# DichenZhang1/libultrahdr_dev

Hardware: AMD Instinct MI355X
Metric: MPixels/sec gain-map generate+apply, 4K P010 batch (higher is better)
Workload: dtype u8/u16 in, f32+f64 math, u8/u32 out

## Files before the change

### libultrahdr_dev_amd/csrc/uhdr_capi.hip

```cpp
#include <hip/hip_runtime.h>

#include <algorithm>
#include <memory>
#include <cmath>
#include <cstdio>
#include <cstring>
#include <map>
#include <chrono>
#include <mutex>
#include <thread>
#include <tuple>
#include <vector>

#include "../../include/uhdr_hip.h"
#include "uhdr_kernels.h"
#include "uhdr_jpeg.h"
#include "uhdr_jpegr.h"

namespace {

using namespace uhdr;

thread_local char t_err[256] = "";

// ... 369 lines not shown
  c.log2_min_d = std::log2((double)md.minContentBoost);
  c.log2_max_d = std::log2((double)md.maxContentBoost);
  c.idw = idw;
  c.lut = nullptr;
  c.lut_boost_factor = c.display_boost > 0 ? c.display_boost / md.maxContentBoost : 1.0f;
  const double lut_top = std::exp2(std::fmax(c.log2_min_d, c.log2_max_d) * (double)c.lut_boost_factor) / (double)c.display_boost;
  c.lut_plain_div = (c.display_boost >= 0x1p-20f && c.display_boost <= 0x1p20f && std::fabs(c.log2_min_d * (double)c.lut_boost_factor) <= 40.0 &&
                     std::fabs(c.log2_max_d * (double)c.lut_boost_factor) <= 40.0 && lut_top <= 32768.0) ? 1u : 0u;
  const double ratio = (double)c.display_boost / (double)md.maxContentBoost;
  c.fast.A = (float)((c.log2_max_d - c.log2_min_d) * ratio);
  c.fast.B = (float)(c.log2_min_d * ratio - std::log2((double)c.display_boost));
  c.fast.A255 = (float)((c.log2_max_d - c.log2_min_d) * ratio / 255.0);
  std::vector<float> t;
  build_idw_tables(4, t);
  for (int oy = 0; oy < 4; ++oy)
    for (int pr = 0; pr < 2; ++pr)
      for (int k = 1; k < 4; ++k)
        for (int j = 0; j < 2; ++j)
          c.fast.wD[oy][pr][k - 1][j] = t[oy * 16 + (2 * pr + j) * 4 + k];
  c.tab = nullptr;
  c.ex_ws = nullptr;
  c.ex_cap = 0;
  c.cells_per_thread = 8;
  c.step_x = c.step_y = 0;
  return c;
}
AppImage app_image(const uhdr_hip_image_t& yuv, const uhdr_hip_image_t& map, void* dst) {
  AppImage a;
  a.y = static_cast<const uint8_t*>(yuv.data);
  a.u = static_cast<const uint8_t*>(yuv.chroma_data);
  a.v = a.u + yuv.chroma_stride * (yuv.height / 2);
  a.map = static_cast<const uint8_t*>(map.data);
  a.dst = dst;
  a.y_stride = (uint32_t)yuv.luma_stride;
  a.c_stride = (uint32_t)yuv.chroma_stride;
  return a;
}
bool app_fast_s4(const AppConsts& c, const AppImage& a) {
  if ((uint64_t)a.y_stride * c.height >= (1ull << 32) || (uint64_t)c.width * c.height >= (1ull << 29)) return false;
  return c.scale == 4 && c.width == 4u * c.map_w && c.height == 4u * c.map_h && al(a.y, 4) && a.y_stride % 4u == 0 &&
         al(a.u, 2) && al(a.v, 2) && a.c_stride % 2u == 0 && al(a.dst, 16);
}
void fill_apply_dest(const uhdr_hip_image_t* yuv, uhdr_hip_image_t* dest) {
  dest->width = yuv->width;
  dest->height = yuv->height;
  dest->colorGamut = yuv->colorGamut;
}
// ... 3485 lines not shown
```

### libultrahdr_dev_amd/csrc/uhdr_kernels.h

```cpp
#pragma once
#include <hip/hip_runtime_api.h>
#include <stdint.h>

namespace uhdr {

constexpr uint32_t kStatSlotWaves = 1024, kStatSlotPlain = 15, kStatSlotSaved = 4, kStatSlotWords = 16 + 16 * kStatSlotSaved;
constexpr uint32_t kStatLists = 64, kStatCap = 252, kStatEst = 8 + kStatLists, kStatSlotCnt = kStatEst + 2 * kStatLists,
                   kStatHdr = kStatSlotCnt + kStatSlotWaves,
                   kStatWords = kStatHdr + (kStatLists * kStatCap > kStatSlotWaves * kStatSlotWords ? kStatLists * kStatCap : kStatSlotWaves * kStatSlotWords);
static_assert(kStatHdr % 4u == 0u && kStatSlotWords % 4u == 0u && kStatWords % 4u == 0u, "saved entries are read and written as 16-byte pieces");
constexpr int kMaxChunk = 64;

constexpr uint32_t kLutSrgbInvN = 1024, kLutHlgInvN = 4096, kLutPqInvN = 4096, kLutHlgN = 65536, kLutPqN = 65536;
constexpr uint32_t kLutSrgbInv = 0, kLutHlgInv = kLutSrgbInv + kLutSrgbInvN, kLutPqInv = kLutHlgInv + kLutHlgInvN,
                   kLutHlg = kLutPqInv + kLutPqInvN, kLutPq = kLutHlg + kLutHlgN, kLutTotal = kLutPq + kLutPqN;
constexpr uint32_t kTabS1Bytes = 0x3C00 + 16;
constexpr uint32_t kTabS1PowBytes = 512u * 8u;
constexpr uint32_t kTabS2Cells = 129, kTabS2Floats = 260;
constexpr uint32_t kTabS2LdsBytes = kTabS2Cells * 256u;
constexpr uint32_t kTabS1Lin = kLutTotal, kTabS1Hlg = kTabS1Lin + kTabS1Bytes / 4, kTabS1Pq = kTabS1Hlg + kTabS1PowBytes / 4,
                   kTabS2Hlg = kTabS1Pq + kTabS1PowBytes / 4, kTabS2Pq = kTabS2Hlg + kTabS2Floats, kTabEnd = kTabS2Pq + kTabS2Floats;
constexpr uint32_t kCodeHlg = kTabEnd, kCodePq = kCodeHlg + kLutHlgN / 2, kLutBufferFloats = kCodePq + kLutPqN / 2;
constexpr uint32_t kGainLutN = 1024;

// ... 25 lines not shown
  uint32_t enc_byte_min, enc_byte_max;
  const float* lut;
  double log2_min_d, log2_max_d;
};
struct GenImage {
  const uint8_t* y;
  const uint8_t* u;
  const uint16_t* hy;
  const uint16_t* huv;
  uint8_t* map;
  uint32_t y_stride, c_stride, hy_stride, huv_stride;
};
struct GenBatch {
  GenImage img[kMaxChunk];
};

struct AppFast {
  float A, B, A255;
  float wD[4][2][3][2];
};
struct AppConsts {
  uint32_t width, height, map_w, map_h, scale;
  uint32_t cells_per_thread;
  uint32_t step_x, step_y;
  float display_boost, inv_display_boost, max_boost, inv_max_boost;
  double log2_min_d, log2_max_d;
  const float* idw;
  const float* lut;
  const float* tab;
  float lut_boost_factor;
  uint32_t lut_plain_div;
  uint32_t* ex_ws;
  uint32_t ex_cap;
  AppFast fast;
};
constexpr uint32_t kExLists = 1024;
constexpr uint32_t kExHdrWords = 8 + kExLists;
inline size_t ex_ws_bytes(uint32_t cap) { return ((size_t)kMaxChunk * kExHdrWords + (size_t)kMaxChunk * kExLists * cap) * 4u; }
inline uint32_t ex_list_cap(uint64_t pixels) { return (uint32_t)(pixels / 16u / kExLists) + 64u; }
struct AppImage {
  const uint8_t* y;
  const uint8_t* u;
  const uint8_t* v;
  const uint8_t* map;
  void* dst;
  uint32_t y_stride, c_stride;
};
// ... 107 lines not shown
```

### libultrahdr_dev_amd/csrc/uhdr_kernels.hip

```cpp
#include "uhdr_kernels.h"

#include <hip/hip_runtime.h>

#include <algorithm>
#include <cmath>

#include "uhdr_device_math.h"
#include "uhdr_wave_scan.h"

namespace uhdr {

__constant__ float c_idw4[4 * 64];

__constant__ float c_idw4p[64];

hipError_t upload_idw4(const float* tables) {
  float p[64];
  for (int oy = 0; oy < 4; ++oy)
    for (int pr = 0; pr < 2; ++pr)
      for (int k = 0; k < 4; ++k)
        for (int h = 0; h < 2; ++h) p[((oy * 2 + pr) * 4 + k) * 2 + h] = tables[oy * 16 + (2 * pr + h) * 4 + k];
  hipError_t e = hipMemcpyToSymbol(HIP_SYMBOL(c_idw4p), p, sizeof(p));
  if (e != hipSuccess) return e;
  return hipMemcpyToSymbol(HIP_SYMBOL(c_idw4), tables, sizeof(float) * 4 * 64);
// ... 277 lines not shown
    out[k] = encode_gain_guarded(gain[k], c.min_boost, c.max_boost, c.log2_min, c.log2_max, c.enc_scale, c.enc_byte_min,
                                 c.enc_byte_max);
  return 3u;
}

typedef uint32_t u32x4 __attribute__((ext_vector_type(4)));
typedef uint32_t u32x2 __attribute__((ext_vector_type(2)));
__device__ __forceinline__ uint4 ld_stream(const uint4* p) {
  const u32x4 v = __builtin_nontemporal_load(reinterpret_cast<const u32x4*>(p));
  return make_uint4(v.x, v.y, v.z, v.w);
}
__device__ __forceinline__ uint2 ld_stream(const uint2* p) {
  const u32x2 v = __builtin_nontemporal_load(reinterpret_cast<const u32x2*>(p));
  return make_uint2(v.x, v.y);
}
__device__ __forceinline__ uint32_t ld_stream(const uint32_t* p) {
  return __builtin_nontemporal_load(p);
}
__device__ __forceinline__ void st_stream(uint4* p, uint4 v) {
  __builtin_nontemporal_store((u32x4){v.x, v.y, v.z, v.w}, reinterpret_cast<u32x4*>(p));
}
__device__ __forceinline__ void st_stream(uint2* p, uint2 v) {
  __builtin_nontemporal_store((u32x2){v.x, v.y}, reinterpret_cast<u32x2*>(p));
}
__device__ __forceinline__ uint32_t ld8(const uint8_t* p) { return *p; }
__device__ __forceinline__ uint32_t ld16(const uint16_t* p) { return *p; }

constexpr int kGenBlock = 256, kGenTiles = 4;

template <bool ALIGNED>
__device__ __forceinline__ void load_pair(const GenConsts& c, const GenImage& im, const uint8_t* im_v, uint32_t my, uint32_t pr,
                                          bool two, uint32_t (&hy)[2][4][2], uint32_t (&huv)[2][2][2], uint32_t (&y8)[2][4],
                                          uint32_t (&u8)[2][2], uint32_t (&v8)[2][2]) {
  const uint32_t mx = pr * 2u;
  if (ALIGNED) {
    const uint32_t hoff = 4u * my * im.hy_stride + 8u * pr, yoff = 4u * my * im.y_stride + 8u * pr;
#pragma unroll
    for (int r = 0; r < 4; ++r) {
      const uint4 q = ld_stream(reinterpret_cast<const uint4*>(im.hy + (hoff + r * im.hy_stride)));
      hy[0][r][0] = q.x; hy[0][r][1] = q.y; hy[1][r][0] = q.z; hy[1][r][1] = q.w;
      const uint2 p = ld_stream(reinterpret_cast<const uint2*>(im.y + (yoff + r * im.y_stride)));
      y8[0][r] = p.x; y8[1][r] = p.y;
    }
    const uint32_t huvoff = 2u * my * im.huv_stride + 8u * pr, coff = 2u * my * im.c_stride + 4u * pr;
#pragma unroll
    for (int r = 0; r < 2; ++r) {
// ... 602 lines not shown
  asm("v_lshl_or_b32 %0, %1, 10, %2" : "=v"(t) : "v"(__float_as_uint(g)), "v"(__float_as_uint(r)));
  asm("v_lshl_or_b32 %0, %1, 20, %2" : "=v"(t) : "v"(__float_as_uint(b)), "v"(t));
  return t;
}

template <int K>
__device__ __forceinline__ float cvt_byte(uint32_t w) { return (float)((w >> (8 * K)) & 0xffu); }

struct PairF { f2 c[3]; f2 factor; float2 e[6]; };
struct PairM { f2 s[3]; float2 e[6]; };
struct ChromaRow { f2 crv, ngs, cbu; };
__device__ __forceinline__ ChromaRow chroma_row(uint32_t uu, uint32_t vv) {
  constexpr float kCrS = kP3Cr * k255, kCbS = kP3Cb * k255, kGCbS = kP3GCb * k255, kGCrS = kP3GCr * k255;
  const f2 uf = (f2){cvt_byte<0>(uu), cvt_byte<1>(uu)};
  const f2 vf = (f2){cvt_byte<0>(vv), cvt_byte<1>(vv)};
  ChromaRow o;
  o.crv = pk_fma(vf, splat(kCrS), splat(-128.0f * kCrS));
  o.cbu = pk_fma(uf, splat(kCbS), splat(-128.0f * kCbS));
  o.ngs = pk_fma(uf, splat(-kGCbS), pk_fma(vf, splat(-kGCrS), splat(128.0f * kGCbS + 128.0f * kGCrS)));
  return o;
}
template <int FMT>
__device__ __forceinline__ void apply_cell_piped(const AppConsts& c, void* dst, uint32_t cx, uint32_t cy,
                                                 const uint32_t (&yrow)[4], const uint32_t (&uu)[2], const uint32_t (&vv)[2],
                                                 float m1, float m2, float m3, float m4, uint32_t slot8, const char* lut) {
  typedef ApplyTab<FMT, false> T;
  ChromaRow cr = chroma_row(uu[0], vv[0]);
  const float a255 = c.fast.A255;
  f2 d23 = (f2){m2 - m1, m3 - m1}, d4b = (f2){m4 - m1, __builtin_fmaf(m1, a255, c.fast.B)};
  asm("" : "+v"(d23), "+v"(d4b));
  PairF pf[2];
  PairM pm[2];
  uint32_t px[4];
#pragma unroll
  for (int k = 0; k < 10; ++k) {
    if (k < 8) {
      const int oy = k >> 1, pr = k & 1;
      const f2 w1 = (f2){c.fast.wD[oy][pr][0][0], c.fast.wD[oy][pr][0][1]}, w2 = (f2){c.fast.wD[oy][pr][1][0], c.fast.wD[oy][pr][1][1]};
      const f2 w3 = (f2){c.fast.wD[oy][pr][2][0], c.fast.wD[oy][pr][2][1]};
      if (k == 4) cr = chroma_row(uu[1], vv[1]);
      PairF& f = pf[k & 1];
      const f2 E = pk_fma(bc_lo(d4b), w3, pk_fma(bc_hi(d23), w2, pk_fma(bc_lo(d23), w1, bc_hi(d4b))));
      const f2 yraw = pr ? (f2){cvt_byte<2>(yrow[oy]), cvt_byte<3>(yrow[oy])} : (f2){cvt_byte<0>(yrow[oy]), cvt_byte<1>(yrow[oy])};
      if (pr) {
        f.c[0] = pk_fma_sat_bc<1>(yraw, splat(k255), cr.crv); f.c[1] = pk_fma_sat_bc<1>(yraw, splat(k255), cr.ngs);
        f.c[2] = pk_fma_sat_bc<1>(yraw, splat(k255), cr.cbu);
      } else {
// ... 14 lines not shown
        asm("v_fma_f32 %0, %1, %2, %3" : "=v"(t.x) : "v"(f.e[2 * ch].y), "v"(f.c[ch].x), "v"(f.e[2 * ch].x));
        asm("v_fma_f32 %0, %1, %2, %3" : "=v"(t.y) : "v"(f.e[2 * ch + 1].y), "v"(f.c[ch].y), "v"(f.e[2 * ch + 1].x));
        m.s[ch] = pk_fma(t, f.factor, splat(2.0f));
      }
#pragma unroll
      for (int ch = 0; ch < 3; ++ch) {
        m.e[2 * ch] = *reinterpret_cast<const float2*>(lut + T::kS2Base + s2_address(m.s[ch].x, slot8));
        m.e[2 * ch + 1] = *reinterpret_cast<const float2*>(lut + T::kS2Base + s2_address(m.s[ch].y, slot8));
      }
    }
    __builtin_amdgcn_sched_barrier(0);
    if (k >= 2) {
      const int q = k - 2, oy = q >> 1, pr = q & 1;
      PairM& m = pm[q & 1];
      float o[6];
#pragma unroll
      for (int ch = 0; ch < 3; ++ch) {
        asm("v_fma_f32 %0, %1, %2, %3" : "=v"(o[2 * ch]) : "v"(m.e[2 * ch].y), "v"(m.s[ch].x), "v"(m.e[2 * ch].x));
        asm("v_fma_f32 %0, %1, %2, %3" : "=v"(o[2 * ch + 1]) : "v"(m.e[2 * ch + 1].y), "v"(m.s[ch].y), "v"(m.e[2 * ch + 1].x));
      }
      px[2 * pr] = pack10_bits(o[0], o[2], o[4]);
      px[2 * pr + 1] = pack10_bits(o[1], o[3], o[5]);
      if (pr) {
        const uint32_t off = ((4u * cy + oy) * c.width + 4u * cx) * 4u;
        st_stream(reinterpret_cast<uint4*>(static_cast<char*>(dst) + off), make_uint4(px[0], px[1], px[2], px[3]));
      }
    }
    __builtin_amdgcn_sched_barrier(0);
  }
}

constexpr uint32_t kXchSecond = 72;
constexpr uint32_t kXchPerWave = 136;
template <int FMT, bool MASK>
__device__ __forceinline__ void apply_cell_piped1(const AppConsts& c, const AppImage& im, uint32_t cx, uint32_t cy,
                                                  const uint32_t (&yrow)[4], const uint32_t (&uu)[2], const uint32_t (&vv)[2],
                                                  float m1, float m2, float m3, float m4, const char* lut, uint4* xch) {
  ChromaRow cr = chroma_row(uu[0], vv[0]);
  const float a255 = c.fast.A255;
  f2 d23 = (f2){m2 - m1, m3 - m1}, d4b = (f2){m4 - m1, __builtin_fmaf(m1, a255, c.fast.B)};
  asm("" : "+v"(d23), "+v"(d4b));
  PairF pf[2];
  PairOut po[2];
  const uint32_t lane = threadIdx.x & 63u;
#pragma unroll
  for (int k = 0; k < 9; ++k) {
    if (k < 8) {
      const int oy = k >> 1, pr = k & 1;
      const f2 w1 = (f2){c.fast.wD[oy][pr][0][0], c.fast.wD[oy][pr][0][1]}, w2 = (f2){c.fast.wD[oy][pr][1][0], c.fast.wD[oy][pr][1][1]};
      const f2 w3 = (f2){c.fast.wD[oy][pr][2][0], c.fast.wD[oy][pr][2][1]};
      if (k == 4) cr = chroma_row(uu[1], vv[1]);
      PairF& f = pf[k & 1];
      const f2 E = pk_fma(bc_lo(d4b), w3, pk_fma(bc_hi(d23), w2, pk_fma(bc_lo(d23), w1, bc_hi(d4b))));
      const f2 yraw = pr ? (f2){cvt_byte<2>(yrow[oy]), cvt_byte<3>(yrow[oy])} : (f2){cvt_byte<0>(yrow[oy]), cvt_byte<1>(yrow[oy])};
      if (pr) {
        f.c[0] = pk_fma_sat_bc<1>(yraw, splat(k255), cr.crv); f.c[1] = pk_fma_sat_bc<1>(yraw, splat(k255), cr.ngs);
        f.c[2] = pk_fma_sat_bc<1>(yraw, splat(k255), cr.cbu);
      } else {
        f.c[0] = pk_fma_sat_bc<0>(yraw, splat(k255), cr.crv); f.c[1] = pk_fma_sat_bc<0>(yraw, splat(k255), cr.ngs);
        f.c[2] = pk_fma_sat_bc<0>(yraw, splat(k255), cr.cbu);
      }
      f.factor = exp2_2(E);
#pragma unroll
      for (int ch = 0; ch < 3; ++ch) tab_pair<0>(f.c[ch], lut, f.e[2 * ch], f.e[2 * ch + 1]);
    }
    __builtin_amdgcn_sched_barrier(0);
    if (k >= 1) {
      const int q = k - 1, oy = q >> 1, pr = q & 1;
      PairF& f = pf[q & 1];
      f2 lin[3];
#pragma unroll
      for (int ch = 0; ch < 3; ++ch) {
        f2 t;
        asm("v_fma_f32 %0, %1, %2, %3" : "=v"(t.x) : "v"(f.e[2 * ch].y), "v"(f.c[ch].x), "v"(f.e[2 * ch].x));
        asm("v_fma_f32 %0, %1, %2, %3" : "=v"(t.y) : "v"(f.e[2 * ch + 1].y), "v"(f.c[ch].y), "v"(f.e[2 * ch + 1].x));
        lin[ch] = oetf2_scaled<FMT>(t * f.factor);
      }
      po[pr].r = lin[0]; po[pr].g = lin[1]; po[pr].b = lin[2];
      if (pr) {
        const uint32_t pix0 = (4u * cy + oy) * c.width + 4u * cx;
        if (FMT == 2 || FMT == 3) {
          uint4 o;
          o.x = pack10_scaled<MASK>(po[0].r.x, po[0].g.x, po[0].b.x); o.y = pack10_scaled<MASK>(po[0].r.y, po[0].g.y, po[0].b.y);
          o.z = pack10_scaled<MASK>(po[1].r.x, po[1].g.x, po[1].b.x); o.w = pack10_scaled<MASK>(po[1].r.y, po[1].g.y, po[1].b.y);
          st_stream(reinterpret_cast<uint4*>(static_cast<uint32_t*>(im.dst) + pix0), o);
        } else if (FMT == 1) {
          const uint2 a = pack_f16_hw(po[0].r.x, po[0].g.x, po[0].b.x), bb = pack_f16_hw(po[0].r.y, po[0].g.y, po[0].b.y);
          const uint2 cc = pack_f16_hw(po[1].r.x, po[1].g.x, po[1].b.x), d = pack_f16_hw(po[1].r.y, po[1].g.y, po[1].b.y);
          if (xch != nullptr) {
            xch[lane] = make_uint4(a.x, a.y, bb.x, bb.y);
            xch[kXchSecond + lane] = make_uint4(cc.x, cc.y, d.x, d.y);
            __builtin_amdgcn_wave_barrier();
            const uint32_t from = (lane & 1u) * kXchSecond + (lane >> 1);
            const uint4 s0 = xch[from], s1 = xch[from + 32u];
            __builtin_amdgcn_wave_barrier();
            uint4* o = reinterpret_cast<uint4*>(static_cast<uint2*>(im.dst) + (uint32_t)__builtin_amdgcn_readfirstlane((int)pix0));
            st_stream(o + lane, s0);
            st_stream(o + 64u + lane, s1);
          } else {
            uint4* o = reinterpret_cast<uint4*>(static_cast<uint2*>(im.dst) + pix0);
            o[0] = make_uint4(a.x, a.y, bb.x, bb.y);
            o[1] = make_uint4(cc.x, cc.y, d.x, d.y);
          }
        } else {
          const size_t plane = (size_t)c.width * c.height;
          uint16_t* base16 = static_cast<uint16_t*>(im.dst);
          const f2 ch[3][2] = {{po[0].r, po[1].r}, {po[0].g, po[1].g}, {po[0].b, po[1].b}};
#pragma unroll
          for (int p = 0; p < 3; ++p) {
            const uint32_t q0 = 0x3ffu & (uint32_t)ch[p][0].x, q1 = 0x3ffu & (uint32_t)ch[p][0].y;
            const uint32_t q2 = 0x3ffu & (uint32_t)ch[p][1].x, q3 = 0x3ffu & (uint32_t)ch[p][1].y;
            st_stream(reinterpret_cast<uint2*>(base16 + p * plane + pix0), make_uint2(q0 | (q1 << 16), q2 | (q3 << 16)));
          }
        }
      }
    }
    __builtin_amdgcn_sched_barrier(0);
  }
}

struct ApplyCellIn { uint32_t yrow[4], uu[2], vv[2], mb[4]; };
__device__ __forceinline__ void apply_load_cell(const AppConsts& c, const AppImage& im, uint32_t cx, uint32_t cy, ApplyCellIn& o) {
  const uint32_t yoff = 4u * cy * im.y_stride + 4u * cx;
#pragma unroll
  for (int r = 0; r < 4; ++r) o.yrow[r] = ld_stream(reinterpret_cast<const uint32_t*>(im.y + (yoff + r * im.y_stride)));
  const uint32_t coff = 2u * cy * im.c_stride + 2u * cx;
#pragma unroll
  for (int r = 0; r < 2; ++r) {
    o.uu[r] = *reinterpret_cast<const uint16_t*>(im.u + (coff + r * im.c_stride));
    o.vv[r] = *reinterpret_cast<const uint16_t*>(im.v + (coff + r * im.c_stride));
  }
  const uint32_t xu = min(cx + 1u, c.map_w - 1u), yu = min(cy + 1u, c.map_h - 1u);
  const uint32_t m0 = cy * c.map_w, m1 = yu * c.map_w;
  o.mb[0] = im.map[m0 + cx]; o.mb[1] = im.map[m1 + cx]; o.mb[2] = im.map[m0 + xu]; o.mb[3] = im.map[m1 + xu];
}

template <int FMT, bool MASK>
__device__ __forceinline__ void apply_cell_edge(const AppConsts& c, const AppImage& im, uint32_t cx, uint32_t cy,
                                                const uint32_t (&yrow)[4], const uint32_t (&uu)[2], const uint32_t (&vv)[2],
                                                float m1, float m2, float m3, float m4, const float* wt ,
                                                uint32_t slot8, const char* lut) {
  typedef ApplyTab<FMT, MASK> T;
  const float a255 = c.fast.A255;
  const float base = __builtin_fmaf(m1, a255, c.fast.B), d2 = m2 - m1, d3 = m3 - m1, d4 = m4 - m1;
#pragma unroll 1
  for (uint32_t oy = 0; oy < 4u; ++oy) {
    const uint32_t yw = oy == 0u ? yrow[0] : oy == 1u ? yrow[1] : oy == 2u ? yrow[2] : yrow[3];
    const ChromaRow cr = chroma_row(oy < 2u ? uu[0] : uu[1], oy < 2u ? vv[0] : vv[1]);
    const uint32_t pix0 = (4u * cy + oy) * c.width + 4u * cx;
    uint32_t px[4];
    PairOut po[2];
#pragma unroll
    for (int pr = 0; pr < 2; ++pr) {
      const f2 yraw = pr ? (f2){cvt_byte<2>(yw), cvt_byte<3>(yw)} : (f2){cvt_byte<0>(yw), cvt_byte<1>(yw)};
      const float* p0 = wt + oy * 16u + pr * 8;
      const f2 w1 = (f2){p0[1], p0[5]}, w2 = (f2){p0[2], p0[6]}, w3 = (f2){p0[3], p0[7]};
      const f2 E = pk_fma(splat(d4), w3, pk_fma(splat(d3), w2, pk_fma(splat(d2), w1, splat(base))));
      const f2 factor = exp2_2(E);
      f2 ch[3];
      if (pr) {
        ch[0] = pk_fma_sat_bc<1>(yraw, splat(k255), cr.crv); ch[1] = pk_fma_sat_bc<1>(yraw, splat(k255), cr.ngs); ch[2] = pk_fma_sat_bc<1>(yraw, splat(k255), cr.cbu);
      } else {
        ch[0] = pk_fma_sat_bc<0>(yraw, splat(k255), cr.crv); ch[1] = pk_fma_sat_bc<0>(yraw, splat(k255), cr.ngs); ch[2] = pk_fma_sat_bc<0>(yraw, splat(k255), cr.cbu);
      }
      if (T::kOetf) {
        float o[6];
#pragma unroll
        for (int q = 0; q < 3; ++q) {
          float2 a, b;
          pow_pair(ch[q], lut, a, b);
          f2 t;
          asm("v_fma_f32 %0, %1, %2, %3" : "=v"(t.x) : "v"(a.y), "v"(ch[q].x), "v"(a.x));
// ... 27 lines not shown
      o.x = pack10_scaled<MASK>(po[0].r.x, po[0].g.x, po[0].b.x); o.y = pack10_scaled<MASK>(po[0].r.y, po[0].g.y, po[0].b.y);
      o.z = pack10_scaled<MASK>(po[1].r.x, po[1].g.x, po[1].b.x); o.w = pack10_scaled<MASK>(po[1].r.y, po[1].g.y, po[1].b.y);
      st_stream(reinterpret_cast<uint4*>(static_cast<uint32_t*>(im.dst) + pix0), o);
    } else if (FMT == 1) {
      const uint2 a = pack_f16_hw(po[0].r.x, po[0].g.x, po[0].b.x), bb = pack_f16_hw(po[0].r.y, po[0].g.y, po[0].b.y);
      const uint2 cc = pack_f16_hw(po[1].r.x, po[1].g.x, po[1].b.x), d = pack_f16_hw(po[1].r.y, po[1].g.y, po[1].b.y);
      uint4* o = reinterpret_cast<uint4*>(static_cast<uint2*>(im.dst) + pix0);
      o[0] = make_uint4(a.x, a.y, bb.x, bb.y);
      o[1] = make_uint4(cc.x, cc.y, d.x, d.y);
    } else {
      const size_t plane = (size_t)c.width * c.height;
      uint16_t* base16 = static_cast<uint16_t*>(im.dst);
      const f2 pl[3][2] = {{po[0].r, po[1].r}, {po[0].g, po[1].g}, {po[0].b, po[1].b}};
#pragma unroll
      for (int p = 0; p < 3; ++p) {
        const uint32_t q0 = 0x3ffu & (uint32_t)pl[p][0].x, q1 = 0x3ffu & (uint32_t)pl[p][0].y;
        const uint32_t q2 = 0x3ffu & (uint32_t)pl[p][1].x, q3 = 0x3ffu & (uint32_t)pl[p][1].y;
        st_stream(reinterpret_cast<uint2*>(base16 + p * plane + pix0), make_uint2(q0 | (q1 << 16), q2 | (q3 << 16)));
      }
    }
  }
}

struct ApplyCellPk { uint32_t yrow[4], uu[2], vv[2], mrow[2]; };
struct __attribute__((packed)) U16Any { uint16_t v; };
__device__ __forceinline__ void apply_load_cell_pk(const AppConsts& c, const AppImage& im, uint32_t cx, uint32_t cy, uint32_t mx, uint32_t cy1, ApplyCellPk& o) {
  const uint32_t yoff = 4u * cy * im.y_stride + 4u * cx;
#pragma unroll
  for (int r = 0; r < 4; ++r) o.yrow[r] = ld_stream(reinterpret_cast<const uint32_t*>(im.y + (yoff + r * im.y_stride)));
  const uint32_t coff = 2u * cy * im.c_stride + 2u * cx;
#pragma unroll
  for (int r = 0; r < 2; ++r) {
    o.uu[r] = *reinterpret_cast<const uint16_t*>(im.u + (coff + r * im.c_stride));
    o.vv[r] = *reinterpret_cast<const uint16_t*>(im.v + (coff + r * im.c_stride));
  }
  o.mrow[0] = reinterpret_cast<const U16Any*>(im.map + (cy * c.map_w + mx))->v;
  o.mrow[1] = reinterpret_cast<const U16Any*>(im.map + (cy1 * c.map_w + mx))->v;
}

constexpr uint32_t kApplyBlock = 512;
constexpr uint32_t kApplyMaxCellsPerThread = 32;

template <int FMT, bool MASK>
__device__ __forceinline__ bool apply_walk_cell(const AppConsts& c, const AppImage& im, uint32_t& cx, uint32_t& cy, uint32_t& left,
                                                const ApplyCellPk& cur, ApplyCellPk& nxt, uint32_t slot8, const char* lut,
                                                const float* s_idw, uint4* s_xch) {
  typedef ApplyTab<FMT, MASK> T;
  uint32_t ncx = cx + c.step_x, ncy = cy + c.step_y;
  if (ncx >= c.map_w) { ncx -= c.map_w; ++ncy; }
  --left;
  const bool more = left != 0u && ncy < c.map_h;
  if (!more) { ncx = cx; ncy = cy; }
  apply_load_cell_pk(c, im, ncx, ncy, ncx - (ncx + 1u == c.map_w ? 1u : 0u), min(ncy + 1u, c.map_h - 1u), nxt);
  const bool edge_x = cx + 1u == c.map_w, edge_y = cy + 1u == c.map_h;
  const float e3 = cvt_byte<1>(cur.mrow[0]), e4 = cvt_byte<1>(cur.mrow[1]);
  const float e1 = edge_x ? e3 : cvt_byte<0>(cur.mrow[0]), e2 = edge_x ? e4 : cvt_byte<0>(cur.mrow[1]);
  const bool interior = __builtin_amdgcn_ballot_w64(edge_x || edge_y) == 0ull;
  const float* wt = s_idw + (edge_x ? (edge_y ? 192 : 64) : (edge_y ? 128 : 0));
  if (T::kOetf) {
    if (interior) apply_cell_piped<FMT>(c, im.dst, cx, cy, cur.yrow, cur.uu, cur.vv, e1, e2, e3, e4, slot8, lut);
    else apply_cell_edge<FMT, MASK>(c, im, cx, cy, cur.yrow, cur.uu, cur.vv, e1, e2, e3, e4, wt, slot8, lut);
  } else {
    uint4* xch = nullptr;
    if (FMT == 1 && __builtin_amdgcn_ballot_w64(true) == ~0ull &&
        __builtin_amdgcn_ballot_w64(cy != (uint32_t)__builtin_amdgcn_readfirstlane((int)cy)) == 0ull)
      xch = s_xch + (threadIdx.x >> 6) * kXchPerWave;
    if (interior) apply_cell_piped1<FMT, MASK>(c, im, cx, cy, cur.yrow, cur.uu, cur.vv, e1, e2, e3, e4, lut, xch);
    else apply_cell_edge<FMT, MASK>(c, im, cx, cy, cur.yrow, cur.uu, cur.vv, e1, e2, e3, e4, wt, slot8, lut);
  }
  cx = ncx; cy = ncy;
  return more;
}

template <int FMT, bool MASK>
__global__ void __launch_bounds__(kApplyBlock, 4) k_apply_s4(const AppConsts c, const AppBatch b) {
  typedef ApplyTab<FMT, MASK> T;
  __shared__ uint4 s_tab[T::kBytes / 16u];
  __shared__ uint4 s_xch[FMT == 1 ? (kApplyBlock / 64) * kXchPerWave : 1];
  __shared__ float s_idw[4 * 64];
  const uint32_t img_i = blockIdx.x, span = blockIdx.y;
  const AppImage& im = b.img[img_i];
  const uint32_t idx = span * c.cells_per_thread * kApplyBlock + threadIdx.x;
  uint32_t cy = idx / c.map_w;
  uint32_t cx = idx - cy * c.map_w;
  const bool any = cy < c.map_h;
  ApplyCellPk ca, cb;
  if (any) apply_load_cell_pk(c, im, cx, cy, cx - (cx + 1u == c.map_w ? 1u : 0u), min(cy + 1u, c.map_h - 1u), ca);
  {
    constexpr uint32_t kN1 = T::kS1Bytes / 16u, kPer1 = (kN1 + kApplyBlock - 1u) / kApplyBlock;
    constexpr uint32_t kN2 = T::kOetf ? kTabS2Cells * 32u : 0u, kPer2 = (kN2 + kApplyBlock - 1u) / kApplyBlock;
    const uint4* src1 = reinterpret_cast<const uint4*>(c.tab + T::kS1Float);
    const uint2* src2 = reinterpret_cast<const uint2*>(c.tab + T::kS2Float);
    uint4 t1[kPer1];
    uint2 t2[kPer2 ? kPer2 : 1u];
    const float w = c_idw4[threadIdx.x & 255u] * c.fast.A255;
#pragma unroll
    for (uint32_t k = 0; k < kPer1; ++k) { const uint32_t i = k * kApplyBlock + threadIdx.x; t1[k] = src1[i < kN1 ? i : kN1 - 1u]; }
#pragma unroll
    for (uint32_t k = 0; k < kPer2; ++k) { const uint32_t i = k * kApplyBlock + threadIdx.x; t2[k] = src2[(i < kN2 ? i : 0u) >> 5]; }
    if (threadIdx.x < 256u) s_idw[threadIdx.x] = w;
#pragma unroll
    for (uint32_t k = 0; k < kPer1; ++k) { const uint32_t i = k * kApplyBlock + threadIdx.x; if (i < kN1) s_tab[i] = t1[k]; }
#pragma unroll
    for (uint32_t k = 0; k < kPer2; ++k) { const uint32_t i = k * kApplyBlock + threadIdx.x; if (i < kN2) reinterpret_cast<uint2*>(s_tab)[T::kS2Base / 8u + i] = t2[k]; }
  }
  __syncthreads();
  const char* lut = reinterpret_cast<const char*>(s_tab);
  const uint32_t slot8 = (threadIdx.x & 31u) << 3;
  if (!any) return;
  if (T::kOetf) {
    asm volatile("s_setreg_imm32_b32 hwreg(HW_REG_MODE, 0, 2), 3" : "+v"(cx), "+v"(cy));
  }
  uint32_t left = c.cells_per_thread;
#pragma unroll 1
  for (;;) {
    if (!apply_walk_cell<FMT, MASK>(c, im, cx, cy, left, ca, cb, slot8, lut, s_idw, s_xch)) return;
    if (!apply_walk_cell<FMT, MASK>(c, im, cx, cy, left, cb, ca, slot8, lut, s_idw, s_xch)) return;
  }
}

struct PxIn { float yf, u, v, gain; };
__device__ __forceinline__ PxIn px_inputs(const AppConsts& c, const AppImage& im, uint32_t x, uint32_t y) {
  PxIn in;
  in.yf = (float)im.y[(size_t)y * im.y_stride + x] * k255;
  const size_t ci = (size_t)(y >> 1) * im.c_stride + (x >> 1);
  in.u = (float)((int)im.u[ci] - 128) * k255;
  in.v = (float)((int)im.v[ci] - 128) * k255;

  const uint32_t s = c.scale;
  uint32_t xl, yl, ox, oy;
  if ((s & (s - 1u)) == 0u) {
    const uint32_t sh = (uint32_t)__builtin_ctz(s);
    xl = x >> sh; yl = y >> sh; ox = x & (s - 1u); oy = y & (s - 1u);
  } else {
    xl = x / s; yl = y / s; ox = x - xl * s; oy = y - yl * s;
  }
  uint32_t xu = xl + 1u, yu = yl + 1u;
  xl = min(xl, c.map_w - 1u); xu = min(xu, c.map_w - 1u);
  yl = min(yl, c.map_h - 1u); yu = min(yu, c.map_h - 1u);
  const float e1 = map_to_float_fast(im.map[(size_t)yl * c.map_w + xl]);
// ... 607 lines not shown
template <int FMT>
static hipError_t launch_apply_t(const AppConsts& c, const AppBatch& b, int n, int mode,
                                 bool fast_s4, hipStream_t s) {
  if (n == 0 || c.width == 0 || c.height == 0) return hipSuccess;
  const bool exact = mode == 1 || mode == 3;
  if (mode == 2) {
    if (c.lut == nullptr) return hipErrorInvalidValue;
    if (fast_s4) {
      constexpr bool kOetf = FMT == 2 || FMT == 3;
      const uint32_t lds = (kOetf ? kLutHlgN * 2u : 0u) + (kLutSrgbInvN + kGainLutN) * 4u;
      const uint32_t chunks = (c.map_w * c.map_h + kLutS4Block - 1u) / kLutS4Block * (uint32_t)n;
      if (hipFuncSetAttribute(reinterpret_cast<const void*>(&k_apply_lut_s4<FMT>), hipFuncAttributeMaxDynamicSharedMemorySize, (int)lds) == hipSuccess) {
        hipLaunchKernelGGL((k_apply_lut_s4<FMT>), dim3(chunks < 256u ? chunks : 256u), dim3(kLutS4Block), lds, s, c, b, (uint32_t)n);
        return hipGetLastError();
      }
      (void)hipGetLastError();
    }
    const size_t total = (size_t)c.width * c.height, per_block = 256u * (size_t)kLutPixelsPerThread;
    hipLaunchKernelGGL((k_apply_lut<FMT>), dim3((unsigned)((total + per_block - 1u) / per_block), n), dim3(256), 0, s, c, b);
    return hipGetLastError();
  }
  if (fast_s4 && !exact && c.map_w >= 2u) {
    AppConsts cc = c;
    const uint32_t total = c.map_w * c.map_h;
    uint32_t cpt = kApplyMaxCellsPerThread;
    auto blocks = [&](uint32_t k) { return (uint64_t)((total + kApplyBlock * k - 1u) / (kApplyBlock * k)) * (uint64_t)n; };
    while (cpt > 1u && blocks(cpt) < 448u) cpt >>= 1;
    cc.cells_per_thread = cpt;
    cc.step_x = kApplyBlock % c.map_w;
    cc.step_y = kApplyBlock / c.map_w;
    const dim3 grid(n, (unsigned)((total + kApplyBlock * cpt - 1u) / (kApplyBlock * cpt)));
    const double top = std::exp2(std::fmax(c.log2_min_d, c.log2_max_d) * (double)c.display_boost / (double)c.max_boost) / (double)c.display_boost;
    const bool mask = !(top <= 1.0 + 1e-6);
    if (!mask && ApplyTab<FMT, false>::kOetf) {
      const float g = FMT == 3 ? 0.5f : UHDR_PQ_M1;
      cc.fast.A *= g; cc.fast.A255 *= g; cc.fast.B = cc.fast.B * g + 1.0f;
    }
    for (int i = 0; i < 4 * 2 * 3 * 2; ++i) (&cc.fast.wD[0][0][0][0])[i] *= cc.fast.A255;
    if (mask) hipLaunchKernelGGL((k_apply_s4<FMT, true>), grid, dim3(kApplyBlock), 0, s, cc, b);
    else hipLaunchKernelGGL((k_apply_s4<FMT, false>), grid, dim3(kApplyBlock), 0, s, cc, b);
  } else {
    const dim3 grid = px_grid(c.width, c.height, n);
    if (exact && c.ex_ws != nullptr) {
      if (fast_s4) hipLaunchKernelGGL((k_apply_s4_est<FMT>), dim3((c.map_w * c.map_h + 255u) / 256u, n), dim3(256), 0, s, c, b);
      else hipLaunchKernelGGL((k_apply_px_est<FMT>), grid, dim3(256), 0, s, c, b);
      hipLaunchKernelGGL((k_apply_resolve<FMT>), dim3(n, kExSlices), dim3(256), 0, s, c, b);
    } else if (exact) hipLaunchKernelGGL((k_apply_px<FMT, true>), grid, dim3(256), 0, s, c, b);
    else hipLaunchKernelGGL((k_apply_px<FMT, false>), grid, dim3(256), 0, s, c, b);
  }
  return hipGetLastError();
}

hipError_t launch_apply(const AppConsts& c, const AppBatch& b, int n, int fmt, int mode,
                        bool fast_s4, hipStream_t s) {
// ... 638 lines not shown
```

Measured before the change: 545,000.

## Walk apply cells down columns and peel right-edge column into dedicated blocks

The scale-4 apply kernel now assigns each thread a fixed map column and walks down a vertical band of cells instead of striding through a flattened cell index. Each step reuses the previous lower gain-map row as the next upper row, and the right-edge column goes to separate edge blocks, so the main loop only checks the bottom edge and drops the per-cell ballot. Row base addresses are forced into scalar registers with 32-bit column offsets, which should cut per-lane address arithmetic. In exchange the grid becomes 3D, extra edge-only blocks are launched, and coalescing now relies on adjacent lanes covering adjacent columns.

```diff
diff --git a/libultrahdr_dev_amd/csrc/uhdr_capi.hip b/libultrahdr_dev_amd/csrc/uhdr_capi.hip
--- a/libultrahdr_dev_amd/csrc/uhdr_capi.hip
+++ b/libultrahdr_dev_amd/csrc/uhdr_capi.hip
@@ -415,7 +415,7 @@
   c.ex_ws = nullptr;
   c.ex_cap = 0;
   c.cells_per_thread = 8;
-  c.step_x = c.step_y = 0;
+  c.strips = c.edge_layers = 0;
   return c;
 }
 AppImage app_image(const uhdr_hip_image_t& yuv, const uhdr_hip_image_t& map, void* dst) {
diff --git a/libultrahdr_dev_amd/csrc/uhdr_kernels.h b/libultrahdr_dev_amd/csrc/uhdr_kernels.h
--- a/libultrahdr_dev_amd/csrc/uhdr_kernels.h
+++ b/libultrahdr_dev_amd/csrc/uhdr_kernels.h
@@ -71,7 +71,7 @@
 struct AppConsts {
   uint32_t width, height, map_w, map_h, scale;
   uint32_t cells_per_thread;
-  uint32_t step_x, step_y;
+  uint32_t strips, edge_layers;
   float display_boost, inv_display_boost, max_boost, inv_max_boost;
   double log2_min_d, log2_max_d;
   const float* idw;
diff --git a/libultrahdr_dev_amd/csrc/uhdr_kernels.hip b/libultrahdr_dev_amd/csrc/uhdr_kernels.hip
--- a/libultrahdr_dev_amd/csrc/uhdr_kernels.hip
+++ b/libultrahdr_dev_amd/csrc/uhdr_kernels.hip
@@ -323,6 +323,22 @@
 }
 __device__ __forceinline__ void st_stream(uint2* p, uint2 v) {
   __builtin_nontemporal_store((u32x2){v.x, v.y}, reinterpret_cast<u32x2*>(p));
+}
+#define UHDR_GLOBAL __attribute__((address_space(1)))
+struct SRow { uint64_t a; };
+__device__ __forceinline__ SRow srow(const void* plane, uint32_t row_bytes) {
+  uint64_t a = reinterpret_cast<uint64_t>(plane) + row_bytes;
+  asm("" : "+s"(a));
+  return SRow{a};
+}
+__device__ __forceinline__ uint32_t ld_stream32(SRow r, uint32_t col) { return __builtin_nontemporal_load((const UHDR_GLOBAL uint32_t*)(r.a + col)); }
+__device__ __forceinline__ uint16_t ld16(SRow r, uint32_t col) { return *(const UHDR_GLOBAL uint16_t*)(r.a + col); }
+__device__ __forceinline__ void st_stream(SRow r, uint32_t col, uint4 v) {
+  __builtin_nontemporal_store((u32x4){v.x, v.y, v.z, v.w}, (UHDR_GLOBAL u32x4*)(r.a + col));
+}
+__device__ __forceinline__ void st_plain(SRow r, uint32_t col, uint4 v) { *(UHDR_GLOBAL u32x4*)(r.a + col) = (u32x4){v.x, v.y, v.z, v.w}; }
+__device__ __forceinline__ void st_stream(SRow r, uint32_t col, uint2 v) {
+  __builtin_nontemporal_store((u32x2){v.x, v.y}, (UHDR_GLOBAL u32x2*)(r.a + col));
 }
 __device__ __forceinline__ uint32_t ld8(const uint8_t* p) { return *p; }
 __device__ __forceinline__ uint32_t ld16(const uint16_t* p) { return *p; }
@@ -971,7 +987,7 @@
 }
 template <int FMT>
 __device__ __forceinline__ void apply_cell_piped(const AppConsts& c, void* dst, uint32_t cx, uint32_t cy,
-                                                 const uint32_t (&yrow)[4], const uint32_t (&uu)[2], const uint32_t (&vv)[2],
+                                                 const uint32_t (&yrow)[4], const uint16_t (&uu)[2], const uint16_t (&vv)[2],
                                                  float m1, float m2, float m3, float m4, uint32_t slot8, const char* lut) {
   typedef ApplyTab<FMT, false> T;
   ChromaRow cr = chroma_row(uu[0], vv[0]);
@@ -1032,8 +1048,7 @@
       px[2 * pr] = pack10_bits(o[0], o[2], o[4]);
       px[2 * pr + 1] = pack10_bits(o[1], o[3], o[5]);
       if (pr) {
-        const uint32_t off = ((4u * cy + oy) * c.width + 4u * cx) * 4u;
-        st_stream(reinterpret_cast<uint4*>(static_cast<char*>(dst) + off), make_uint4(px[0], px[1], px[2], px[3]));
+        st_stream(srow(dst, (4u * cy + oy) * c.width * 4u), 16u * cx, make_uint4(px[0], px[1], px[2], px[3]));
       }
     }
     __builtin_amdgcn_sched_barrier(0);
@@ -1044,7 +1059,7 @@
 constexpr uint32_t kXchPerWave = 136;
 template <int FMT, bool MASK>
 __device__ __forceinline__ void apply_cell_piped1(const AppConsts& c, const AppImage& im, uint32_t cx, uint32_t cy,
-                                                  const uint32_t (&yrow)[4], const uint32_t (&uu)[2], const uint32_t (&vv)[2],
+                                                  const uint32_t (&yrow)[4], const uint16_t (&uu)[2], const uint16_t (&vv)[2],
                                                   float m1, float m2, float m3, float m4, const char* lut, uint4* xch) {
   ChromaRow cr = chroma_row(uu[0], vv[0]);
   const float a255 = c.fast.A255;
@@ -1088,12 +1103,12 @@
       }
       po[pr].r = lin[0]; po[pr].g = lin[1]; po[pr].b = lin[2];
       if (pr) {
-        const uint32_t pix0 = (4u * cy + oy) * c.width + 4u * cx;
+        const uint32_t row0 = (4u * cy + oy) * c.width, col0 = 4u * cx;
         if (FMT == 2 || FMT == 3) {
           uint4 o;
           o.x = pack10_scaled<MASK>(po[0].r.x, po[0].g.x, po[0].b.x); o.y = pack10_scaled<MASK>(po[0].r.y, po[0].g.y, po[0].b.y);
           o.z = pack10_scaled<MASK>(po[1].r.x, po[1].g.x, po[1].b.x); o.w = pack10_scaled<MASK>(po[1].r.y, po[1].g.y, po[1].b.y);
-          st_stream(reinterpret_cast<uint4*>(static_cast<uint32_t*>(im.dst) + pix0), o);
+          st_stream(srow(im.dst, 4u * row0), 4u * col0, o);
         } else if (FMT == 1) {
           const uint2 a = pack_f16_hw(po[0].r.x, po[0].g.x, po[0].b.x), bb = pack_f16_hw(po[0].r.y, po[0].g.y, po[0].b.y);
           const uint2 cc = pack_f16_hw(po[1].r.x, po[1].g.x, po[1].b.x), d = pack_f16_hw(po[1].r.y, po[1].g.y, po[1].b.y);
@@ -1104,13 +1119,13 @@
             const uint32_t from = (lane & 1u) * kXchSecond + (lane >> 1);
             const uint4 s0 = xch[from], s1 = xch[from + 32u];
             __builtin_amdgcn_wave_barrier();
-            uint4* o = reinterpret_cast<uint4*>(static_cast<uint2*>(im.dst) + (uint32_t)__builtin_amdgcn_readfirstlane((int)pix0));
-            st_stream(o + lane, s0);
-            st_stream(o + 64u + lane, s1);
+            const SRow o = srow(im.dst, 8u * (row0 + (uint32_t)__builtin_amdgcn_readfirstlane((int)col0)));
+            st_stream(o, 16u * lane, s0);
+            st_stream(o, 16u * (64u + lane), s1);
           } else {
-            uint4* o = reinterpret_cast<uint4*>(static_cast<uint2*>(im.dst) + pix0);
-            o[0] = make_uint4(a.x, a.y, bb.x, bb.y);
-            o[1] = make_uint4(cc.x, cc.y, d.x, d.y);
+            const SRow o = srow(im.dst, 8u * row0);
+            st_plain(o, 8u * col0, make_uint4(a.x, a.y, bb.x, bb.y));
+            st_plain(o, 8u * col0 + 16u, make_uint4(cc.x, cc.y, d.x, d.y));
           }
         } else {
           const size_t plane = (size_t)c.width * c.height;
@@ -1120,7 +1135,7 @@
           for (int p = 0; p < 3; ++p) {
             const uint32_t q0 = 0x3ffu & (uint32_t)ch[p][0].x, q1 = 0x3ffu & (uint32_t)ch[p][0].y;
             const uint32_t q2 = 0x3ffu & (uint32_t)ch[p][1].x, q3 = 0x3ffu & (uint32_t)ch[p][1].y;
-            st_stream(reinterpret_cast<uint2*>(base16 + p * plane + pix0), make_uint2(q0 | (q1 << 16), q2 | (q3 << 16)));
+            st_stream(srow(base16 + p * plane, 2u * row0), 2u * col0, make_uint2(q0 | (q1 << 16), q2 | (q3 << 16)));
           }
         }
       }
@@ -1147,7 +1162,7 @@
 
 template <int FMT, bool MASK>
 __device__ __forceinline__ void apply_cell_edge(const AppConsts& c, const AppImage& im, uint32_t cx, uint32_t cy,
-                                                const uint32_t (&yrow)[4], const uint32_t (&uu)[2], const uint32_t (&vv)[2],
+                                                const uint32_t (&yrow)[4], const uint16_t (&uu)[2], const uint16_t (&vv)[2],
                                                 float m1, float m2, float m3, float m4, const float* wt ,
                                                 uint32_t slot8, const char* lut) {
   typedef ApplyTab<FMT, MASK> T;
@@ -1157,7 +1172,7 @@
   for (uint32_t oy = 0; oy < 4u; ++oy) {
     const uint32_t yw = oy == 0u ? yrow[0] : oy == 1u ? yrow[1] : oy == 2u ? yrow[2] : yrow[3];
     const ChromaRow cr = chroma_row(oy < 2u ? uu[0] : uu[1], oy < 2u ? vv[0] : vv[1]);
-    const uint32_t pix0 = (4u * cy + oy) * c.width + 4u * cx;
+    const size_t pix0 = (size_t)((4u * cy + oy) * c.width) + (size_t)(4u * cx);
     uint32_t px[4];
     PairOut po[2];
 #pragma unroll
@@ -1231,53 +1246,57 @@
   }
 }
 
-struct ApplyCellPk { uint32_t yrow[4], uu[2], vv[2], mrow[2]; };
+struct ApplyCol { uint32_t yrow[4]; uint16_t uu[2], vv[2], mlo; };
 struct __attribute__((packed)) U16Any { uint16_t v; };
-__device__ __forceinline__ void apply_load_cell_pk(const AppConsts& c, const AppImage& im, uint32_t cx, uint32_t cy, uint32_t mx, uint32_t cy1, ApplyCellPk& o) {
-  const uint32_t yoff = 4u * cy * im.y_stride + 4u * cx;
-#pragma unroll
-  for (int r = 0; r < 4; ++r) o.yrow[r] = ld_stream(reinterpret_cast<const uint32_t*>(im.y + (yoff + r * im.y_stride)));
-  const uint32_t coff = 2u * cy * im.c_stride + 2u * cx;
-#pragma unroll
-  for (int r = 0; r < 2; ++r) {
-    o.uu[r] = *reinterpret_cast<const uint16_t*>(im.u + (coff + r * im.c_stride));
-    o.vv[r] = *reinterpret_cast<const uint16_t*>(im.v + (coff + r * im.c_stride));
-  }
-  o.mrow[0] = reinterpret_cast<const U16Any*>(im.map + (cy * c.map_w + mx))->v;
-  o.mrow[1] = reinterpret_cast<const U16Any*>(im.map + (cy1 * c.map_w + mx))->v;
+__device__ __forceinline__ uint16_t apply_load_map_row(const AppConsts& c, const AppImage& im, uint32_t mx, uint32_t row) {
+  return reinterpret_cast<const U16Any*>(im.map + (size_t)(row * c.map_w) + (size_t)mx)->v;
+}
+__device__ __forceinline__ void apply_load_col(const AppConsts& c, const AppImage& im, uint32_t cx, uint32_t cy, uint32_t mx, uint32_t cy1, ApplyCol& o) {
+#pragma unroll
+  for (uint32_t r = 0; r < 4u; ++r) o.yrow[r] = ld_stream(reinterpret_cast<const uint32_t*>(im.y + (size_t)((4u * cy + r) * im.y_stride) + (size_t)(4u * cx)));
+#pragma unroll
+  for (uint32_t r = 0; r < 2u; ++r) {
+    const size_t coff = (2u * cy + r) * im.c_stride;
+    o.uu[r] = *reinterpret_cast<const uint16_t*>(im.u + coff + (size_t)(2u * cx));
+    o.vv[r] = *reinterpret_cast<const uint16_t*>(im.v + coff + (size_t)(2u * cx));
+  }
+  o.mlo = apply_load_map_row(c, im, mx, cy1);
+}
+__device__ __forceinline__ void apply_load_col_s(const AppConsts& c, const AppImage& im, uint32_t cx, uint32_t cy, uint32_t cy1, ApplyCol& o) {
+#pragma unroll
+  for (uint32_t r = 0; r < 4u; ++r) o.yrow[r] = ld_stream32(srow(im.y, (4u * cy + r) * im.y_stride), 4u * cx);
+#pragma unroll
+  for (uint32_t r = 0; r < 2u; ++r) {
+    o.uu[r] = ld16(srow(im.u, (2u * cy + r) * im.c_stride), 2u * cx);
+    o.vv[r] = ld16(srow(im.v, (2u * cy + r) * im.c_stride), 2u * cx);
+  }
+  o.mlo = ((const UHDR_GLOBAL U16Any*)(srow(im.map, cy1 * c.map_w).a + cx))->v;
 }
 
 constexpr uint32_t kApplyBlock = 512;
 constexpr uint32_t kApplyMaxCellsPerThread = 32;
 
 template <int FMT, bool MASK>
-__device__ __forceinline__ bool apply_walk_cell(const AppConsts& c, const AppImage& im, uint32_t& cx, uint32_t& cy, uint32_t& left,
-                                                const ApplyCellPk& cur, ApplyCellPk& nxt, uint32_t slot8, const char* lut,
-                                                const float* s_idw, uint4* s_xch) {
+__device__ __forceinline__ bool apply_walk_cell(const AppConsts& c, const AppImage& im, uint32_t cx, uint32_t& cy, uint32_t& left,
+                                                uint16_t& mup, const ApplyCol& cur, ApplyCol& nxt, uint32_t slot8, const char* lut,
+                                                const float* s_idw, uint4* xch) {
   typedef ApplyTab<FMT, MASK> T;
-  uint32_t ncx = cx + c.step_x, ncy = cy + c.step_y;
-  if (ncx >= c.map_w) { ncx -= c.map_w; ++ncy; }
+  asm volatile("" : "+v"(cx));
   --left;
-  const bool more = left != 0u && ncy < c.map_h;
-  if (!more) { ncx = cx; ncy = cy; }
-  apply_load_cell_pk(c, im, ncx, ncy, ncx - (ncx + 1u == c.map_w ? 1u : 0u), min(ncy + 1u, c.map_h - 1u), nxt);
-  const bool edge_x = cx + 1u == c.map_w, edge_y = cy + 1u == c.map_h;
-  const float e3 = cvt_byte<1>(cur.mrow[0]), e4 = cvt_byte<1>(cur.mrow[1]);
-  const float e1 = edge_x ? e3 : cvt_byte<0>(cur.mrow[0]), e2 = edge_x ? e4 : cvt_byte<0>(cur.mrow[1]);
-  const bool interior = __builtin_amdgcn_ballot_w64(edge_x || edge_y) == 0ull;
-  const float* wt = s_idw + (edge_x ? (edge_y ? 192 : 64) : (edge_y ? 128 : 0));
+  const bool more = left != 0u;
+  const uint32_t ncy = more ? cy + 1u : cy;
+  apply_load_col_s(c, im, cx, ncy, min(ncy + 1u, c.map_h - 1u), nxt);
+  const float e1 = cvt_byte<0>(mup), e3 = cvt_byte<1>(mup), e2 = cvt_byte<0>(cur.mlo), e4 = cvt_byte<1>(cur.mlo);
+  mup = cur.mlo;
+  const bool edge_y = cy + 1u == c.map_h;
   if (T::kOetf) {
-    if (interior) apply_cell_piped<FMT>(c, im.dst, cx, cy, cur.yrow, cur.uu, cur.vv, e1, e2, e3, e4, slot8, lut);
-    else apply_cell_edge<FMT, MASK>(c, im, cx, cy, cur.yrow, cur.uu, cur.vv, e1, e2, e3, e4, wt, slot8, lut);
+    if (!edge_y) apply_cell_piped<FMT>(c, im.dst, cx, cy, cur.yrow, cur.uu, cur.vv, e1, e2, e3, e4, slot8, lut);
+    else apply_cell_edge<FMT, MASK>(c, im, cx, cy, cur.yrow, cur.uu, cur.vv, e1, e2, e3, e4, s_idw + 128, slot8, lut);
   } else {
-    uint4* xch = nullptr;
-    if (FMT == 1 && __builtin_amdgcn_ballot_w64(true) == ~0ull &&
-        __builtin_amdgcn_ballot_w64(cy != (uint32_t)__builtin_amdgcn_readfirstlane((int)cy)) == 0ull)
-      xch = s_xch + (threadIdx.x >> 6) * kXchPerWave;
-    if (interior) apply_cell_piped1<FMT, MASK>(c, im, cx, cy, cur.yrow, cur.uu, cur.vv, e1, e2, e3, e4, lut, xch);
-    else apply_cell_edge<FMT, MASK>(c, im, cx, cy, cur.yrow, cur.uu, cur.vv, e1, e2, e3, e4, wt, slot8, lut);
-  }
-  cx = ncx; cy = ncy;
+    if (!edge_y) apply_cell_piped1<FMT, MASK>(c, im, cx, cy, cur.yrow, cur.uu, cur.vv, e1, e2, e3, e4, lut, xch);
+    else apply_cell_edge<FMT, MASK>(c, im, cx, cy, cur.yrow, cur.uu, cur.vv, e1, e2, e3, e4, s_idw + 128, slot8, lut);
+  }
+  cy = ncy;
   return more;
 }
 
@@ -1287,14 +1306,22 @@
   __shared__ uint4 s_tab[T::kBytes / 16u];
   __shared__ uint4 s_xch[FMT == 1 ? (kApplyBlock / 64) * kXchPerWave : 1];
   __shared__ float s_idw[4 * 64];
-  const uint32_t img_i = blockIdx.x, span = blockIdx.y;
-  const AppImage& im = b.img[img_i];
-  const uint32_t idx = span * c.cells_per_thread * kApplyBlock + threadIdx.x;
-  uint32_t cy = idx / c.map_w;
-  uint32_t cx = idx - cy * c.map_w;
-  const bool any = cy < c.map_h;
-  ApplyCellPk ca, cb;
-  if (any) apply_load_cell_pk(c, im, cx, cy, cx - (cx + 1u == c.map_w ? 1u : 0u), min(cy + 1u, c.map_h - 1u), ca);
+  const AppImage& im = b.img[blockIdx.x];
+  const uint32_t last = c.map_w - 1u;
+  const bool edge_blk = blockIdx.z < c.edge_layers;
+  const uint32_t band_y = (blockIdx.z - c.edge_layers) * c.cells_per_thread;
+  const uint32_t edge_y0 = (blockIdx.z * c.strips + blockIdx.y) * kApplyBlock;
+  if (edge_blk && edge_y0 >= c.map_h) return;
+  uint32_t cx = edge_blk ? last : blockIdx.y * kApplyBlock + threadIdx.x;
+  uint32_t ey = edge_blk ? edge_y0 + threadIdx.x : band_y;
+  const bool any = edge_blk ? ey < c.map_h : cx < last;
+  ApplyCol ca, cb;
+  uint16_t mup = 0u;
+  if (any) {
+    const uint32_t mx = edge_blk ? last - 1u : cx;
+    mup = apply_load_map_row(c, im, mx, ey);
+    apply_load_col(c, im, cx, ey, mx, min(ey + 1u, c.map_h - 1u), ca);
+  }
   {
     constexpr uint32_t kN1 = T::kS1Bytes / 16u, kPer1 = (kN1 + kApplyBlock - 1u) / kApplyBlock;
     constexpr uint32_t kN2 = T::kOetf ? kTabS2Cells * 32u : 0u, kPer2 = (kN2 + kApplyBlock - 1u) / kApplyBlock;
@@ -1318,13 +1345,24 @@
   const uint32_t slot8 = (threadIdx.x & 31u) << 3;
   if (!any) return;
   if (T::kOetf) {
-    asm volatile("s_setreg_imm32_b32 hwreg(HW_REG_MODE, 0, 2), 3" : "+v"(cx), "+v"(cy));
-  }
-  uint32_t left = c.cells_per_thread;
+    asm volatile("s_setreg_imm32_b32 hwreg(HW_REG_MODE, 0, 2), 3"
+                 : "+v"(cx), "+v"(ey), "+v"(mup), "+v"(ca.mlo), "+v"(ca.yrow[0]), "+v"(ca.yrow[1]), "+v"(ca.yrow[2]), "+v"(ca.yrow[3]),
+                   "+v"(ca.uu[0]), "+v"(ca.uu[1]), "+v"(ca.vv[0]), "+v"(ca.vv[1]));
+  }
+  if (edge_blk) {
+    const float e3 = cvt_byte<1>(mup), e4 = cvt_byte<1>(ca.mlo);
+    const float* wt = s_idw + (ey + 1u == c.map_h ? 192 : 64);
+    apply_cell_edge<FMT, MASK>(c, im, cx, ey, ca.yrow, ca.uu, ca.vv, e3, e4, e3, e4, wt, slot8, lut);
+    return;
+  }
+  uint4* xch = nullptr;
+  if (FMT == 1 && __builtin_amdgcn_ballot_w64(true) == ~0ull) xch = s_xch + (threadIdx.x >> 6) * kXchPerWave;
+  uint32_t cy = band_y;
+  uint32_t left = min(c.cells_per_thread, c.map_h - band_y);
 #pragma unroll 1
   for (;;) {
-    if (!apply_walk_cell<FMT, MASK>(c, im, cx, cy, left, ca, cb, slot8, lut, s_idw, s_xch)) return;
-    if (!apply_walk_cell<FMT, MASK>(c, im, cx, cy, left, cb, ca, slot8, lut, s_idw, s_xch)) return;
+    if (!apply_walk_cell<FMT, MASK>(c, im, cx, cy, left, mup, ca, cb, slot8, lut, s_idw, xch)) return;
+    if (!apply_walk_cell<FMT, MASK>(c, im, cx, cy, left, mup, cb, ca, slot8, lut, s_idw, xch)) return;
   }
 }
 
@@ -1978,14 +2016,16 @@
   }
   if (fast_s4 && !exact && c.map_w >= 2u) {
     AppConsts cc = c;
-    const uint32_t total = c.map_w * c.map_h;
+    const uint32_t strips = (c.map_w - 1u + kApplyBlock - 1u) / kApplyBlock;
     uint32_t cpt = kApplyMaxCellsPerThread;
-    auto blocks = [&](uint32_t k) { return (uint64_t)((total + kApplyBlock * k - 1u) / (kApplyBlock * k)) * (uint64_t)n; };
-    while (cpt > 1u && blocks(cpt) < 448u) cpt >>= 1;
+    auto bands = [&](uint32_t k) { return (c.map_h + k - 1u) / k; };
+    while (cpt > 1u && (uint64_t)strips * bands(cpt) * (uint64_t)n < 448u) cpt >>= 1;
+    const uint32_t edge_blocks = (c.map_h + kApplyBlock - 1u) / kApplyBlock;
+    cc.edge_layers = (edge_blocks + strips - 1u) / strips;
+    while (bands(cpt) + cc.edge_layers > 65535u) cpt <<= 1;
     cc.cells_per_thread = cpt;
-    cc.step_x = kApplyBlock % c.map_w;
-    cc.step_y = kApplyBlock / c.map_w;
-    const dim3 grid(n, (unsigned)((total + kApplyBlock * cpt - 1u) / (kApplyBlock * cpt)));
+    cc.strips = strips;
+    const dim3 grid(n, strips, cc.edge_layers + bands(cpt));
     const double top = std::exp2(std::fmax(c.log2_min_d, c.log2_max_d) * (double)c.display_boost / (double)c.max_boost) / (double)c.display_boost;
     const bool mask = !(top <= 1.0 + 1e-6);
     if (!mask && ApplyTab<FMT, false>::kOetf) {
```

After: 539,100. 0.989x the previous value.
